# AnyLoc/AnyLoc

Hardware: NVIDIA H100
Metric: images/sec end-to-end DINOv2-VLAD descriptors (higher is better)
Workload: dtype f32-equivalent (tensor-core fp16 3-term split, fp32 accumulate)

## Files before the change

anyloc_b200/csrc/attention_wg.cu:

```cuda
#include <stdlib.h>
#include "tc_common.cuh"

namespace anyloc {
namespace awg {

using namespace tc;

__device__ __forceinline__ float ex2(float x) {
  float y; asm("ex2.approx.ftz.f32 %0, %1;" : "=f"(y) : "f"(x)); return y;
}

constexpr int BQ = 128, BKV = 64, HD = 64, THREADS = 384, STAGES = 4;
constexpr int TILE_BYTES = 64 * 128;

template <int FMT> struct Cfg {
  static constexpr int NT = Fmt<FMT>::LO ? 2 : 1;
  static constexpr int Q_BYTES = NT * 2 * TILE_BYTES;
  static constexpr int K_OFF = 0, V_OFF = NT * TILE_BYTES;
  static constexpr int STAGE_BYTES = 2 * NT * TILE_BYTES;
  static constexpr int BAR_OFF = Q_BYTES + STAGES * STAGE_BYTES;
  static constexpr int SMEM_BYTES = BAR_OFF + 256 + 1024 ;
};

template <int FMT, bool VARLEN>
__device__ __forceinline__ void attention_wg_cta(const CUtensorMap* tm_hi, const CUtensorMap* tm_lo, int T, int D,
                                                 void* __restrict__ o_hi_, void* __restrict__ o_lo_,
                                                 const VarlenAttnTable* tab) {
  using C = Cfg<FMT>;
  using F = Fmt<FMT>;
  constexpr bool PAIRS = F::LO;
  extern __shared__ uint8_t smem_raw[];
  uint8_t* smem = reinterpret_cast<uint8_t*>((reinterpret_cast<uintptr_t>(smem_raw) + 1023) & ~(uintptr_t)1023);
  uint64_t* full_bar = reinterpret_cast<uint64_t*>(smem + C::BAR_OFF);
  uint64_t* empty_bar = full_bar + STAGES;
  uint64_t* q_bar = empty_bar + STAGES;

  int qt = blockIdx.x;
  const int h = blockIdx.y;
  int img = blockIdx.z, row0 = 0;
  size_t out0 = (size_t)blockIdx.z * T;
  if constexpr (VARLEN) {
    int lo = 0, hi = tab->n - 1;
    while (lo < hi) {
      const int mid = (lo + hi + 1) >> 1;
      if (tab->tile0[mid] <= qt) lo = mid; else hi = mid - 1;
    }
    qt -= tab->tile0[lo]; T = tab->len[lo]; row0 = tab->row0[lo]; img = 0; out0 = (size_t)row0;
  }
  const int nblk = (T + BKV - 1) / BKV;
  const int active = min(2, (T - qt * BQ + 63) / 64);
  const int wg = threadIdx.x >> 7;

  if (threadIdx.x == 0) {
    asm volatile("prefetch.tensormap [%0];" ::"l"(tm_hi) : "memory");
    for (int s = 0; s < STAGES; ++s) { mbar_init(smem_u32(full_bar + s), 1); mbar_init(smem_u32(empty_bar + s), active); }
    mbar_init(smem_u32(q_bar), 1);
    asm volatile("fence.mbarrier_init.release.cluster;" ::: "memory");
  }
  __syncthreads();

  if (wg == 0) {
    setmaxnreg_dec<24>();
    if (threadIdx.x == 0) {
      const uint32_t qb = smem_u32(q_bar);
      mbar_expect_tx(qb, C::Q_BYTES);
      for (int a = 0; a < C::NT; ++a)
        for (int r = 0; r < 2; ++r)
          tma_load_3d(smem_u32(smem + (2 * a + r) * TILE_BYTES), a ? tm_lo : tm_hi, qb, h * HD,
                      row0 + qt * BQ + 64 * r, img);
      for (int j = 0; j < nblk; ++j) {
        const int stage = j % STAGES;
        mbar_wait(smem_u32(empty_bar + stage), ((j / STAGES) & 1) ^ 1);
        const uint32_t fb = smem_u32(full_bar + stage);
        mbar_expect_tx(fb, C::STAGE_BYTES);
        const uint32_t sb = smem_u32(smem + C::Q_BYTES + stage * C::STAGE_BYTES);
        for (int a = 0; a < C::NT; ++a) {
          tma_load_3d(sb + C::K_OFF + a * TILE_BYTES, a ? tm_lo : tm_hi, fb, D + h * HD, row0 + j * BKV, img);
          tma_load_3d(sb + C::V_OFF + a * TILE_BYTES, a ? tm_lo : tm_hi, fb, 2 * D + h * HD, row0 + j * BKV, img);
        }
      }
    }
    return;
  }

  setmaxnreg_inc<240>();
  const int cw = wg - 1;
  if (qt * BQ + cw * 64 >= T) return;
  const int t = threadIdx.x & 127, warp = t >> 5, lane = t & 31, g = lane >> 2, t4 = lane & 3;
  constexpr bool SCALED = F::SCALED;
  const float P_SCALE = SCALED ? 1024.0f : 1.0f;
  const float kScale = 0.125f * 1.4426950408889634f * (SCALED ? 1.0f / (kActScale * kActScale) : 1.0f);
  auto logit = [&](float s) {
    if constexpr (SCALED) return fmaf(s, kScale, s * 0.0f);
    else return s * kScale;
  };

  const uint32_t q_base = smem_u32(smem) + cw * TILE_BYTES;
  const uint64_t dq_hi = make_desc(q_base), dq_lo = make_desc(q_base + 2 * TILE_BYTES);
  auto stage_addr = [&](int j) { return smem_u32(smem + C::Q_BYTES + (j % STAGES) * C::STAGE_BYTES); };

  auto issue_s = [&](float* s, int j) {
    const uint32_t sb = stage_addr(j);
    const uint64_t dk_hi = make_desc(sb + C::K_OFF), dk_lo = make_desc(sb + C::K_OFF + TILE_BYTES);
    fence_regs<32>(s);
    wgmma_fence();
#pragma unroll
    for (int k = 0; k < 4; ++k) {
      const uint64_t adv = (uint64_t)((k * 32) >> 4);
      wgmma_m64n64_ss<FMT>(s, dq_hi + adv, dk_hi + adv, k != 0 ? 1u : 0u);
      if constexpr (PAIRS) {
        wgmma_m64n64_ss<FMT>(s, dq_lo + adv, dk_hi + adv, 1u);
        wgmma_m64n64_ss<FMT>(s, dq_hi + adv, dk_lo + adv, 1u);
      }
    }
    wgmma_commit();
    fence_regs<32>(s);
  };

  float o[32];
#pragma unroll
  for (int i = 0; i < 32; ++i) o[i] = 0.f;
  float m0 = -INFINITY, m1 = -INFINITY, l0 = 0.f, l1 = 0.f;

  auto block = [&](float* sc, float* sn, int j) {
    if (j + 1 < nblk) {
      mbar_wait(smem_u32(full_bar + (j + 1) % STAGES), ((j + 1) / STAGES) & 1);
      issue_s(sn, j + 1);
    }
    float p[32];
#pragma unroll
    for (int i = 0; i < 32; ++i) p[i] = sc[i];
    float mx0 = m0, mx1 = m1;
#pragma unroll
    for (int nt = 0; nt < 8; ++nt) {
      const int key = j * BKV + nt * 8 + 2 * t4;
#pragma unroll
      for (int e = 0; e < 2; ++e) {
        const bool live = key + e < T;
        p[4 * nt + e] = live ? logit(p[4 * nt + e]) : -INFINITY;
        p[4 * nt + 2 + e] = live ? logit(p[4 * nt + 2 + e]) : -INFINITY;
        mx0 = fmaxf(mx0, p[4 * nt + e]); mx1 = fmaxf(mx1, p[4 * nt + 2 + e]);
      }
    }
    mx0 = fmaxf(mx0, __shfl_xor_sync(0xffffffffu, mx0, 1)); mx0 = fmaxf(mx0, __shfl_xor_sync(0xffffffffu, mx0, 2));
    mx1 = fmaxf(mx1, __shfl_xor_sync(0xffffffffu, mx1, 1)); mx1 = fmaxf(mx1, __shfl_xor_sync(0xffffffffu, mx1, 2));
    const float alpha0 = ex2(m0 - mx0), alpha1 = ex2(m1 - mx1);
    m0 = mx0; m1 = mx1;
    float r0 = 0.f, r1 = 0.f;
#pragma unroll
    for (int nt = 0; nt < 8; ++nt) {
      p[4 * nt + 0] = ex2(p[4 * nt + 0] - mx0); p[4 * nt + 1] = ex2(p[4 * nt + 1] - mx0);
      p[4 * nt + 2] = ex2(p[4 * nt + 2] - mx1); p[4 * nt + 3] = ex2(p[4 * nt + 3] - mx1);
      r0 += p[4 * nt + 0] + p[4 * nt + 1]; r1 += p[4 * nt + 2] + p[4 * nt + 3];
    }
    l0 = l0 * alpha0 + r0; l1 = l1 * alpha1 + r1;

    uint32_t ph[4][4], pl[4][4];
#pragma unroll
    for (int ks = 0; ks < 4; ++ks) {
#pragma unroll
      for (int i = 0; i < 4; ++i) {
        F::pack2(p[8 * ks + 2 * i] * P_SCALE, p[8 * ks + 2 * i + 1] * P_SCALE, ph[ks][i], pl[ks][i]);
      }
    }
    const uint32_t sb = stage_addr(j);
    if constexpr (VARLEN) {
      const int rem = T - j * BKV;
      if (rem < BKV) {
        const int pieces = (BKV - rem) * 8;
        for (int i = cw * 128 + t; i < C::NT * pieces; i += active * 128) {
          const int a = i / pieces, r = rem + (i % pieces) / 8;
          asm volatile("st.shared.v4.u32 [%0], {%1, %1, %1, %1};" ::"r"(sb + C::V_OFF + a * TILE_BYTES + r * 128 +
                                                                          (i % 8) * 16), "r"(0u) : "memory");
        }
        fence_proxy_async_smem();
        named_bar_sync<1>(active * 128);
      }
    }
    const uint64_t dv_hi = make_desc_mn(sb + C::V_OFF), dv_lo = make_desc_mn(sb + C::V_OFF + TILE_BYTES);
    float pv[32];
#pragma unroll
    for (int i = 0; i < 32; ++i) pv[i] = 0.f;
    fence_regs<32>(pv);
    wgmma_fence();
#pragma unroll
    for (int ks = 0; ks < 4; ++ks) {
      const uint64_t adv = (uint64_t)((ks * 2048) >> 4);
      wgmma_m64n64_rs_tb<FMT>(pv, ph[ks], dv_hi + adv, ks != 0 ? 1u : 0u);
      if constexpr (PAIRS) {
        wgmma_m64n64_rs_tb<FMT>(pv, pl[ks], dv_hi + adv, 1u);
        wgmma_m64n64_rs_tb<FMT>(pv, ph[ks], dv_lo + adv, 1u);
      }
    }
    wgmma_commit();
    fence_regs<32>(pv);
    wgmma_wait<0>();
    fence_regs<32>(pv);
    fence_regs<32>(sn);
    if (t == 0) mbar_arrive(smem_u32(empty_bar + j % STAGES));
#pragma unroll
    for (int nd = 0; nd < 8; ++nd) {
      o[4 * nd + 0] = o[4 * nd + 0] * alpha0 + pv[4 * nd + 0]; o[4 * nd + 1] = o[4 * nd + 1] * alpha0 + pv[4 * nd + 1];
      o[4 * nd + 2] = o[4 * nd + 2] * alpha1 + pv[4 * nd + 2]; o[4 * nd + 3] = o[4 * nd + 3] * alpha1 + pv[4 * nd + 3];
    }
  };

  float sa[32], sb[32];
  mbar_wait(smem_u32(q_bar), 0);
  mbar_wait(smem_u32(full_bar), 0);
  issue_s(sa, 0);
  wgmma_wait<0>();
  fence_regs<32>(sa);
  for (int j = 0; j < nblk; j += 2) {
    block(sa, sb, j);
    if (j + 1 < nblk) block(sb, sa, j + 1);
  }

  l0 += __shfl_xor_sync(0xffffffffu, l0, 1); l0 += __shfl_xor_sync(0xffffffffu, l0, 2);
  l1 += __shfl_xor_sync(0xffffffffu, l1, 1); l1 += __shfl_xor_sync(0xffffffffu, l1, 2);
  const float inv0 = 1.0f / (l0 * P_SCALE), inv1 = 1.0f / (l1 * P_SCALE);
  const int q0 = qt * BQ + cw * 64 + warp * 16 + g;
#pragma unroll
  for (int half = 0; half < 2; ++half) {
    const int q = q0 + 8 * half;
    if (q >= T) continue;
    const float inv = half ? inv1 : inv0;
    const size_t off = (out0 + q) * (size_t)D + (size_t)h * HD + 2 * t4;
#pragma unroll
    for (int nd = 0; nd < 8; ++nd) {
      uint32_t hh, ll;
      F::pack2(o[4 * nd + 2 * half] * inv, o[4 * nd + 2 * half + 1] * inv, hh, ll);
      *reinterpret_cast<uint32_t*>(reinterpret_cast<typename F::T*>(o_hi_) + off + nd * 8) = hh;
      if constexpr (F::LO) *reinterpret_cast<uint32_t*>(reinterpret_cast<typename F::T*>(o_lo_) + off + nd * 8) = ll;
    }
  }
}

template <int FMT>
__global__ void __launch_bounds__(THREADS, 1)
attention_wg_kernel(const __grid_constant__ CUtensorMap tm_hi, const __grid_constant__ CUtensorMap tm_lo, int T, int D,
                    void* __restrict__ o_hi, void* __restrict__ o_lo) {
  attention_wg_cta<FMT, false>(&tm_hi, &tm_lo, T, D, o_hi, o_lo, nullptr);
}

template <int FMT>
__global__ void __launch_bounds__(THREADS, 1)
attention_wg_varlen_kernel(const __grid_constant__ CUtensorMap tm_hi, const __grid_constant__ CUtensorMap tm_lo,
                           const __grid_constant__ VarlenAttnTable tab, int D, void* __restrict__ o_hi,
                           void* __restrict__ o_lo) {
  attention_wg_cta<FMT, true>(&tm_hi, &tm_lo, 0, D, o_hi, o_lo, &tab);
}

static int launch(const void* qkv_hi, const void* qkv_lo, int imgs, int rows, int T, const VarlenAttnTable* tab,
                  dim3 grid, int D, void* o_hi, void* o_lo, int fmt, cudaStream_t st) {
  CUtensorMap m_hi, m_lo;
  int rc;
  if ((rc = tc::make_map_3d16(&m_hi, qkv_hi, imgs, rows, 3 * D, 64, fmt))) return rc;
  if ((rc = tc::make_map_3d16(&m_lo, format_info(fmt).lo ? qkv_lo : qkv_hi, imgs, rows, 3 * D, 64, fmt))) return rc;
  return fmt_switch(fmt, [&](auto c) {
    constexpr int FMT = decltype(c)::value;
    if constexpr (sizeof(typename Fmt<FMT>::T) != 2) {
      set_error("attention_wg: format %d is not a 2-byte format", fmt);
      return (int)ANYLOC_ERR_ARG;
    } else {
      static unsigned long long seen = 0;
      if (first_use_on_this_device(&seen)) {
        ANYLOC_CHECK_CUDA(cudaFuncSetAttribute(attention_wg_kernel<FMT>, cudaFuncAttributeMaxDynamicSharedMemorySize,
                                               Cfg<FMT>::SMEM_BYTES));
        ANYLOC_CHECK_CUDA(cudaFuncSetAttribute(attention_wg_varlen_kernel<FMT>,
                                               cudaFuncAttributeMaxDynamicSharedMemorySize, Cfg<FMT>::SMEM_BYTES));
      }
      if (tab)
        attention_wg_varlen_kernel<FMT><<<grid, THREADS, Cfg<FMT>::SMEM_BYTES, st>>>(m_hi, m_lo, *tab, D, o_hi, o_lo);
      else
        attention_wg_kernel<FMT><<<grid, THREADS, Cfg<FMT>::SMEM_BYTES, st>>>(m_hi, m_lo, T, D, o_hi, o_lo);
      ANYLOC_CHECK_LAUNCH();
      return (int)ANYLOC_OK;
    }
  });
}

}

int attention_wg_launch(const void* qkv_hi, const void* qkv_lo, int B, int T, int D, int heads, void* o_hi, void* o_lo,
                        int fmt, cudaStream_t st) {
  using namespace awg;
  return launch(qkv_hi, qkv_lo, B, T, T, nullptr, dim3(cdiv(T, BQ), heads, B), D, o_hi, o_lo, fmt, st);
}

int attention_wg_varlen_launch(const void* qkv_hi, const void* qkv_lo, const VarlenAttnTable& tab, int D, int heads,
                               void* o_hi, void* o_lo, int fmt, cudaStream_t st) {
  using namespace awg;
  VarlenAttnTable t = tab;
  int tiles = 0, rows = 0;
  for (int k = 0; k < t.n; ++k) {
    t.tile0[k] = tiles;
    tiles += cdiv(t.len[k], BQ);
    if (t.row0[k] + t.len[k] > rows) rows = t.row0[k] + t.len[k];
  }
  return launch(qkv_hi, qkv_lo, 1, rows, 0, &t, dim3(tiles, heads), D, o_hi, o_lo, fmt, st);
}

}
```

anyloc_b200/csrc/tc_common.cuh:

```cuda
#pragma once
#include <cuda.h>
#include "formats.cuh"

namespace anyloc {
namespace tc {

__device__ __forceinline__ uint32_t smem_u32(const void* p) { return (uint32_t)__cvta_generic_to_shared(p); }

__device__ __forceinline__ void mbar_init(uint32_t bar, uint32_t count) {
  asm volatile("mbarrier.init.shared::cta.b64 [%0], %1;" ::"r"(bar), "r"(count));
}
__device__ __forceinline__ void mbar_expect_tx(uint32_t bar, uint32_t bytes) {
  asm volatile("mbarrier.arrive.expect_tx.shared::cta.b64 _, [%0], %1;" ::"r"(bar), "r"(bytes) : "memory");
}
__device__ __forceinline__ void mbar_arrive(uint32_t bar) {
  asm volatile("mbarrier.arrive.shared::cta.b64 _, [%0];" ::"r"(bar) : "memory");
}
__device__ __forceinline__ void mbar_wait(uint32_t bar, uint32_t parity) {
  uint32_t done = 0;
  long long t0 = 0;
  for (uint32_t it = 0; !done; ++it) {
    asm volatile(
        "{\n\t.reg .pred p;\n\t"
        "mbarrier.try_wait.parity.shared::cta.b64 p, [%1], %2;\n\t"
        "selp.u32 %0, 1, 0, p;\n\t}"
        : "=r"(done) : "r"(bar), "r"(parity) : "memory");
    if (!done && (it & 0x3ff) == 0x3ff) {
      long long now = clock64();
      if (t0 == 0) t0 = now;
      else if (now - t0 > 8000000000LL) __trap();
    }
  }
}
__device__ __forceinline__ void tma_load_2d(uint32_t dst, const CUtensorMap* map, uint32_t bar, int c0, int c1) {
  asm volatile(
      "cp.async.bulk.tensor.2d.shared::cluster.global.mbarrier::complete_tx::bytes [%0], [%1, {%3, %4}], [%2];"
      ::"r"(dst), "l"(map), "r"(bar), "r"(c0), "r"(c1) : "memory");
}

__device__ __forceinline__ void tma_store_2d(const CUtensorMap* map, uint32_t src, int c0, int c1) {
  asm volatile("cp.async.bulk.tensor.2d.global.shared::cta.bulk_group [%0, {%2, %3}], [%1];"
               ::"l"(map), "r"(src), "r"(c0), "r"(c1) : "memory");
}
__device__ __forceinline__ void bulk_commit() { asm volatile("cp.async.bulk.commit_group;" ::: "memory"); }
template <int N>
__device__ __forceinline__ void bulk_wait_read() { asm volatile("cp.async.bulk.wait_group.read %0;" ::"n"(N) : "memory"); }
template <int N>
__device__ __forceinline__ void bulk_wait() { asm volatile("cp.async.bulk.wait_group %0;" ::"n"(N) : "memory"); }
__device__ __forceinline__ void fence_proxy_async_smem() { asm volatile("fence.proxy.async.shared::cta;" ::: "memory"); }
template <int ID>
__device__ __forceinline__ void named_bar_sync(int count) {
  asm volatile("bar.sync %0, %1;" ::"n"(ID), "r"(count) : "memory");
}

__device__ __forceinline__ uint64_t make_desc(uint32_t saddr) {
  uint64_t d = 0;
  d |= (uint64_t)((saddr & 0x3FFFF) >> 4);
  d |= (uint64_t)1 << 16;
  d |= (uint64_t)(1024 >> 4) << 32;
  d |= (uint64_t)1 << 62;
  return d;
}

__device__ __forceinline__ void wgmma_fence() { asm volatile("wgmma.fence.sync.aligned;" ::: "memory"); }
__device__ __forceinline__ void wgmma_commit() { asm volatile("wgmma.commit_group.sync.aligned;" ::: "memory"); }
template <int N>
__device__ __forceinline__ void wgmma_wait() { asm volatile("wgmma.wait_group.sync.aligned %0;" ::"n"(N) : "memory"); }
template <int R>
__device__ __forceinline__ void fence_regs(float* d) {
#pragma unroll
  for (int i = 0; i < R; ++i) asm volatile("" : "+f"(d[i])::"memory");
}

#define ANYLOC_WG_D64                                                                                               \
  "+f"(d[0]), "+f"(d[1]), "+f"(d[2]), "+f"(d[3]), "+f"(d[4]), "+f"(d[5]), "+f"(d[6]), "+f"(d[7]), "+f"(d[8]),       \
      "+f"(d[9]), "+f"(d[10]), "+f"(d[11]), "+f"(d[12]), "+f"(d[13]), "+f"(d[14]), "+f"(d[15]), "+f"(d[16]),        \
      "+f"(d[17]), "+f"(d[18]), "+f"(d[19]), "+f"(d[20]), "+f"(d[21]), "+f"(d[22]), "+f"(d[23]), "+f"(d[24]),       \
      "+f"(d[25]), "+f"(d[26]), "+f"(d[27]), "+f"(d[28]), "+f"(d[29]), "+f"(d[30]), "+f"(d[31]), "+f"(d[32]),       \
      "+f"(d[33]), "+f"(d[34]), "+f"(d[35]), "+f"(d[36]), "+f"(d[37]), "+f"(d[38]), "+f"(d[39]), "+f"(d[40]),       \
      "+f"(d[41]), "+f"(d[42]), "+f"(d[43]), "+f"(d[44]), "+f"(d[45]), "+f"(d[46]), "+f"(d[47]), "+f"(d[48]),       \
      "+f"(d[49]), "+f"(d[50]), "+f"(d[51]), "+f"(d[52]), "+f"(d[53]), "+f"(d[54]), "+f"(d[55]), "+f"(d[56]),       \
      "+f"(d[57]), "+f"(d[58]), "+f"(d[59]), "+f"(d[60]), "+f"(d[61]), "+f"(d[62]), "+f"(d[63])
#define ANYLOC_WG_D64_STR                                                                                           \
  "{%0, %1, %2, %3, %4, %5, %6, %7, %8, %9, %10, %11, %12, %13, %14, %15, %16, %17, %18, %19, %20, %21, %22, %23, " \
  "%24, %25, %26, %27, %28, %29, %30, %31, %32, %33, %34, %35, %36, %37, %38, %39, %40, %41, %42, %43, %44, %45, "  \
  "%46, %47, %48, %49, %50, %51, %52, %53, %54, %55, %56, %57, %58, %59, %60, %61, %62, %63}"
#define ANYLOC_WG_M64N128(SHAPE_TYPES, TAIL)                                                                        \
  asm volatile("{\n\t.reg .pred p;\n\tsetp.ne.b32 p, %66, 0;\n\t"                                                 \
               "wgmma.mma_async.sync.aligned.m64n128" SHAPE_TYPES " " ANYLOC_WG_D64_STR ", %64, %65, p, 1, 1" TAIL     \
               ";\n\t}"                                                                                              \
               : ANYLOC_WG_D64 : "l"(adesc), "l"(bdesc), "r"(scale_d))

template <int FMT>
__device__ __forceinline__ void wgmma_m64n128(float* d, uint64_t adesc, uint64_t bdesc, uint32_t scale_d) {
  if constexpr (FMT == ANYLOC_PAIR_TF32) ANYLOC_WG_M64N128("k8.f32.tf32.tf32", "");
  else if constexpr (FMT == ANYLOC_PAIR_FP8) ANYLOC_WG_M64N128("k32.f32.e4m3.e4m3", "");
  else if constexpr (FMT == ANYLOC_PAIR_BF16) ANYLOC_WG_M64N128("k16.f32.bf16.bf16", ", 0, 0");
  else ANYLOC_WG_M64N128("k16.f32.f16.f16", ", 0, 0");
}
#undef ANYLOC_WG_M64N128
#undef ANYLOC_WG_D64
#undef ANYLOC_WG_D64_STR

__device__ __forceinline__ void tma_load_3d(uint32_t dst, const CUtensorMap* map, uint32_t bar, int c0, int c1, int c2) {
  asm volatile(
      "cp.async.bulk.tensor.3d.shared::cluster.global.mbarrier::complete_tx::bytes [%0], [%1, {%3, %4, %5}], [%2];"
      ::"r"(dst), "l"(map), "r"(bar), "r"(c0), "r"(c1), "r"(c2) : "memory");
}

template <int N> __device__ __forceinline__ void setmaxnreg_dec() { asm volatile("setmaxnreg.dec.sync.aligned.u32 %0;" ::"n"(N)); }
template <int N> __device__ __forceinline__ void setmaxnreg_inc() { asm volatile("setmaxnreg.inc.sync.aligned.u32 %0;" ::"n"(N)); }

__device__ __forceinline__ uint64_t make_desc_mn(uint32_t saddr) {
  uint64_t d = 0;
  d |= (uint64_t)((saddr & 0x3FFFF) >> 4);
  d |= (uint64_t)(1024 >> 4) << 16;
  d |= (uint64_t)(1024 >> 4) << 32;
  d |= (uint64_t)1 << 62;
  return d;
}

#define ANYLOC_WG_D32                                                                                               \
  "+f"(d[0]), "+f"(d[1]), "+f"(d[2]), "+f"(d[3]), "+f"(d[4]), "+f"(d[5]), "+f"(d[6]), "+f"(d[7]), "+f"(d[8]),       \
      "+f"(d[9]), "+f"(d[10]), "+f"(d[11]), "+f"(d[12]), "+f"(d[13]), "+f"(d[14]), "+f"(d[15]), "+f"(d[16]),        \
      "+f"(d[17]), "+f"(d[18]), "+f"(d[19]), "+f"(d[20]), "+f"(d[21]), "+f"(d[22]), "+f"(d[23]), "+f"(d[24]),       \
      "+f"(d[25]), "+f"(d[26]), "+f"(d[27]), "+f"(d[28]), "+f"(d[29]), "+f"(d[30]), "+f"(d[31])
#define ANYLOC_WG_D32_STR                                                                                           \
  "{%0, %1, %2, %3, %4, %5, %6, %7, %8, %9, %10, %11, %12, %13, %14, %15, %16, %17, %18, %19, %20, %21, %22, %23, " \
  "%24, %25, %26, %27, %28, %29, %30, %31}"

template <int FMT>
__device__ __forceinline__ void wgmma_m64n64_ss(float* d, uint64_t adesc, uint64_t bdesc, uint32_t scale_d) {
  if constexpr (FMT == ANYLOC_PAIR_BF16)
    asm volatile("{\n\t.reg .pred p;\n\tsetp.ne.b32 p, %34, 0;\n\t"
                 "wgmma.mma_async.sync.aligned.m64n64k16.f32.bf16.bf16 " ANYLOC_WG_D32_STR ", %32, %33, p, 1, 1, 0, 0;\n\t}"
                 : ANYLOC_WG_D32 : "l"(adesc), "l"(bdesc), "r"(scale_d));
  else
    asm volatile("{\n\t.reg .pred p;\n\tsetp.ne.b32 p, %34, 0;\n\t"
                 "wgmma.mma_async.sync.aligned.m64n64k16.f32.f16.f16 " ANYLOC_WG_D32_STR ", %32, %33, p, 1, 1, 0, 0;\n\t}"
                 : ANYLOC_WG_D32 : "l"(adesc), "l"(bdesc), "r"(scale_d));
}

template <int FMT>
__device__ __forceinline__ void wgmma_m64n64_rs_tb(float* d, const uint32_t* a, uint64_t bdesc, uint32_t scale_d) {
  if constexpr (FMT == ANYLOC_PAIR_BF16)
    asm volatile("{\n\t.reg .pred p;\n\tsetp.ne.b32 p, %37, 0;\n\t"
                 "wgmma.mma_async.sync.aligned.m64n64k16.f32.bf16.bf16 " ANYLOC_WG_D32_STR
                 ", {%32, %33, %34, %35}, %36, p, 1, 1, 1;\n\t}"
                 : ANYLOC_WG_D32 : "r"(a[0]), "r"(a[1]), "r"(a[2]), "r"(a[3]), "l"(bdesc), "r"(scale_d));
  else
    asm volatile("{\n\t.reg .pred p;\n\tsetp.ne.b32 p, %37, 0;\n\t"
                 "wgmma.mma_async.sync.aligned.m64n64k16.f32.f16.f16 " ANYLOC_WG_D32_STR
                 ", {%32, %33, %34, %35}, %36, p, 1, 1, 1;\n\t}"
                 : ANYLOC_WG_D32 : "r"(a[0]), "r"(a[1]), "r"(a[2]), "r"(a[3]), "l"(bdesc), "r"(scale_d));
}
#undef ANYLOC_WG_D32
#undef ANYLOC_WG_D32_STR

int make_map(CUtensorMap* map, const void* ptr, int rows, int K, int ld, int box_rows, int fmt);
int make_map_3d16(CUtensorMap* map, const void* ptr, int imgs, int rows, int cols, int box_rows, int fmt);

}
}
```

Before: 179.0.

## Hold Q in registers and defer PV wait to overlap with next softmax

Loads the Q tile once into registers with ldmatrix and switches the QK^T wgmma from shared-memory A operands to register A operands. It also restructures the flash-attention loop so the PV wgmma of block j is not waited on immediately. The output accumulation for block j is deferred into block j+1, after the next S result is ready, so PV matmul overlaps with the next softmax. This adds register pressure from 32 extra Q registers and a persistent pv buffer, and makes the stage-release timing more delicate.

```diff
diff --git a/anyloc_b200/csrc/attention_wg.cu b/anyloc_b200/csrc/attention_wg.cu
--- a/anyloc_b200/csrc/attention_wg.cu
+++ b/anyloc_b200/csrc/attention_wg.cu
@@ -95,9 +95,20 @@
     else return s * kScale;
   };
 
-  const uint32_t q_base = smem_u32(smem) + cw * TILE_BYTES;
-  const uint64_t dq_hi = make_desc(q_base), dq_lo = make_desc(q_base + 2 * TILE_BYTES);
   auto stage_addr = [&](int j) { return smem_u32(smem + C::Q_BYTES + (j % STAGES) * C::STAGE_BYTES); };
+
+  uint32_t qh[4][4], ql[4][4];
+  mbar_wait(smem_u32(q_bar), 0);
+  {
+    const int r = warp * 16 + (lane & 7) + ((lane >> 3) & 1) * 8;
+    const uint32_t q_row = smem_u32(smem) + cw * TILE_BYTES + r * 128;
+#pragma unroll
+    for (int ks = 0; ks < 4; ++ks) {
+      const uint32_t off = (uint32_t)(((2 * ks + (lane >> 4)) ^ (r & 7)) << 4);
+      ldsm_x4(qh[ks], q_row + off);
+      if constexpr (PAIRS) ldsm_x4(ql[ks], q_row + 2 * TILE_BYTES + off);
+    }
+  }
 
   auto issue_s = [&](float* s, int j) {
     const uint32_t sb = stage_addr(j);
@@ -107,10 +118,10 @@
 #pragma unroll
     for (int k = 0; k < 4; ++k) {
       const uint64_t adv = (uint64_t)((k * 32) >> 4);
-      wgmma_m64n64_ss<FMT>(s, dq_hi + adv, dk_hi + adv, k != 0 ? 1u : 0u);
+      wgmma_m64n64_rs<FMT, 0>(s, qh[k], dk_hi + adv, k != 0 ? 1u : 0u);
       if constexpr (PAIRS) {
-        wgmma_m64n64_ss<FMT>(s, dq_lo + adv, dk_hi + adv, 1u);
-        wgmma_m64n64_ss<FMT>(s, dq_hi + adv, dk_lo + adv, 1u);
+        wgmma_m64n64_rs<FMT, 0>(s, ql[k], dk_hi + adv, 1u);
+        wgmma_m64n64_rs<FMT, 0>(s, qh[k], dk_lo + adv, 1u);
       }
     }
     wgmma_commit();
@@ -118,15 +129,32 @@
   };
 
   float o[32];
+  float pv[32];
 #pragma unroll
   for (int i = 0; i < 32; ++i) o[i] = 0.f;
   float m0 = -INFINITY, m1 = -INFINITY, l0 = 0.f, l1 = 0.f;
+  float alpha0 = 1.f, alpha1 = 1.f;
+
+  auto update_o = [&](int j) {
+    fence_regs<32>(pv);
+    if (t == 0) mbar_arrive(smem_u32(empty_bar + j % STAGES));
+#pragma unroll
+    for (int nd = 0; nd < 8; ++nd) {
+      o[4 * nd + 0] = o[4 * nd + 0] * alpha0 + pv[4 * nd + 0]; o[4 * nd + 1] = o[4 * nd + 1] * alpha0 + pv[4 * nd + 1];
+      o[4 * nd + 2] = o[4 * nd + 2] * alpha1 + pv[4 * nd + 2]; o[4 * nd + 3] = o[4 * nd + 3] * alpha1 + pv[4 * nd + 3];
+    }
+  };
 
   auto block = [&](float* sc, float* sn, int j) {
     if (j + 1 < nblk) {
       mbar_wait(smem_u32(full_bar + (j + 1) % STAGES), ((j + 1) / STAGES) & 1);
       issue_s(sn, j + 1);
-    }
+      wgmma_wait<1>();
+    } else {
+      wgmma_wait<0>();
+    }
+    fence_regs<32>(sc);
+    if (j > 0) update_o(j - 1);
     float p[32];
 #pragma unroll
     for (int i = 0; i < 32; ++i) p[i] = sc[i];
@@ -144,7 +172,7 @@
     }
     mx0 = fmaxf(mx0, __shfl_xor_sync(0xffffffffu, mx0, 1)); mx0 = fmaxf(mx0, __shfl_xor_sync(0xffffffffu, mx0, 2));
     mx1 = fmaxf(mx1, __shfl_xor_sync(0xffffffffu, mx1, 1)); mx1 = fmaxf(mx1, __shfl_xor_sync(0xffffffffu, mx1, 2));
-    const float alpha0 = ex2(m0 - mx0), alpha1 = ex2(m1 - mx1);
+    alpha0 = ex2(m0 - mx0); alpha1 = ex2(m1 - mx1);
     m0 = mx0; m1 = mx1;
     float r0 = 0.f, r1 = 0.f;
 #pragma unroll
@@ -178,7 +206,6 @@
       }
     }
     const uint64_t dv_hi = make_desc_mn(sb + C::V_OFF), dv_lo = make_desc_mn(sb + C::V_OFF + TILE_BYTES);
-    float pv[32];
 #pragma unroll
     for (int i = 0; i < 32; ++i) pv[i] = 0.f;
     fence_regs<32>(pv);
@@ -186,35 +213,25 @@
 #pragma unroll
     for (int ks = 0; ks < 4; ++ks) {
       const uint64_t adv = (uint64_t)((ks * 2048) >> 4);
-      wgmma_m64n64_rs_tb<FMT>(pv, ph[ks], dv_hi + adv, ks != 0 ? 1u : 0u);
+      wgmma_m64n64_rs<FMT, 1>(pv, ph[ks], dv_hi + adv, ks != 0 ? 1u : 0u);
       if constexpr (PAIRS) {
-        wgmma_m64n64_rs_tb<FMT>(pv, pl[ks], dv_hi + adv, 1u);
-        wgmma_m64n64_rs_tb<FMT>(pv, ph[ks], dv_lo + adv, 1u);
+        wgmma_m64n64_rs<FMT, 1>(pv, pl[ks], dv_hi + adv, 1u);
+        wgmma_m64n64_rs<FMT, 1>(pv, ph[ks], dv_lo + adv, 1u);
       }
     }
     wgmma_commit();
     fence_regs<32>(pv);
-    wgmma_wait<0>();
-    fence_regs<32>(pv);
-    fence_regs<32>(sn);
-    if (t == 0) mbar_arrive(smem_u32(empty_bar + j % STAGES));
-#pragma unroll
-    for (int nd = 0; nd < 8; ++nd) {
-      o[4 * nd + 0] = o[4 * nd + 0] * alpha0 + pv[4 * nd + 0]; o[4 * nd + 1] = o[4 * nd + 1] * alpha0 + pv[4 * nd + 1];
-      o[4 * nd + 2] = o[4 * nd + 2] * alpha1 + pv[4 * nd + 2]; o[4 * nd + 3] = o[4 * nd + 3] * alpha1 + pv[4 * nd + 3];
-    }
   };
 
   float sa[32], sb[32];
-  mbar_wait(smem_u32(q_bar), 0);
   mbar_wait(smem_u32(full_bar), 0);
   issue_s(sa, 0);
-  wgmma_wait<0>();
-  fence_regs<32>(sa);
   for (int j = 0; j < nblk; j += 2) {
     block(sa, sb, j);
     if (j + 1 < nblk) block(sb, sa, j + 1);
   }
+  wgmma_wait<0>();
+  update_o(nblk - 1);
 
   l0 += __shfl_xor_sync(0xffffffffu, l0, 1); l0 += __shfl_xor_sync(0xffffffffu, l0, 2);
   l1 += __shfl_xor_sync(0xffffffffu, l1, 1); l1 += __shfl_xor_sync(0xffffffffu, l1, 2);
diff --git a/anyloc_b200/csrc/tc_common.cuh b/anyloc_b200/csrc/tc_common.cuh
--- a/anyloc_b200/csrc/tc_common.cuh
+++ b/anyloc_b200/csrc/tc_common.cuh
@@ -129,30 +129,23 @@
   "{%0, %1, %2, %3, %4, %5, %6, %7, %8, %9, %10, %11, %12, %13, %14, %15, %16, %17, %18, %19, %20, %21, %22, %23, " \
   "%24, %25, %26, %27, %28, %29, %30, %31}"
 
-template <int FMT>
-__device__ __forceinline__ void wgmma_m64n64_ss(float* d, uint64_t adesc, uint64_t bdesc, uint32_t scale_d) {
-  if constexpr (FMT == ANYLOC_PAIR_BF16)
-    asm volatile("{\n\t.reg .pred p;\n\tsetp.ne.b32 p, %34, 0;\n\t"
-                 "wgmma.mma_async.sync.aligned.m64n64k16.f32.bf16.bf16 " ANYLOC_WG_D32_STR ", %32, %33, p, 1, 1, 0, 0;\n\t}"
-                 : ANYLOC_WG_D32 : "l"(adesc), "l"(bdesc), "r"(scale_d));
-  else
-    asm volatile("{\n\t.reg .pred p;\n\tsetp.ne.b32 p, %34, 0;\n\t"
-                 "wgmma.mma_async.sync.aligned.m64n64k16.f32.f16.f16 " ANYLOC_WG_D32_STR ", %32, %33, p, 1, 1, 0, 0;\n\t}"
-                 : ANYLOC_WG_D32 : "l"(adesc), "l"(bdesc), "r"(scale_d));
-}
-
-template <int FMT>
-__device__ __forceinline__ void wgmma_m64n64_rs_tb(float* d, const uint32_t* a, uint64_t bdesc, uint32_t scale_d) {
+template <int FMT, int TRANS_B>
+__device__ __forceinline__ void wgmma_m64n64_rs(float* d, const uint32_t* a, uint64_t bdesc, uint32_t scale_d) {
   if constexpr (FMT == ANYLOC_PAIR_BF16)
     asm volatile("{\n\t.reg .pred p;\n\tsetp.ne.b32 p, %37, 0;\n\t"
                  "wgmma.mma_async.sync.aligned.m64n64k16.f32.bf16.bf16 " ANYLOC_WG_D32_STR
-                 ", {%32, %33, %34, %35}, %36, p, 1, 1, 1;\n\t}"
-                 : ANYLOC_WG_D32 : "r"(a[0]), "r"(a[1]), "r"(a[2]), "r"(a[3]), "l"(bdesc), "r"(scale_d));
+                 ", {%32, %33, %34, %35}, %36, p, 1, 1, %38;\n\t}"
+                 : ANYLOC_WG_D32 : "r"(a[0]), "r"(a[1]), "r"(a[2]), "r"(a[3]), "l"(bdesc), "r"(scale_d), "n"(TRANS_B));
   else
     asm volatile("{\n\t.reg .pred p;\n\tsetp.ne.b32 p, %37, 0;\n\t"
                  "wgmma.mma_async.sync.aligned.m64n64k16.f32.f16.f16 " ANYLOC_WG_D32_STR
-                 ", {%32, %33, %34, %35}, %36, p, 1, 1, 1;\n\t}"
-                 : ANYLOC_WG_D32 : "r"(a[0]), "r"(a[1]), "r"(a[2]), "r"(a[3]), "l"(bdesc), "r"(scale_d));
+                 ", {%32, %33, %34, %35}, %36, p, 1, 1, %38;\n\t}"
+                 : ANYLOC_WG_D32 : "r"(a[0]), "r"(a[1]), "r"(a[2]), "r"(a[3]), "l"(bdesc), "r"(scale_d), "n"(TRANS_B));
+}
+
+__device__ __forceinline__ void ldsm_x4(uint32_t* r, uint32_t saddr) {
+  asm volatile("ldmatrix.sync.aligned.m8n8.x4.shared.b16 {%0, %1, %2, %3}, [%4];"
+               : "=r"(r[0]), "=r"(r[1]), "=r"(r[2]), "=r"(r[3]) : "r"(saddr) : "memory");
 }
 #undef ANYLOC_WG_D32
 #undef ANYLOC_WG_D32_STR
```

After: 179.4, median of 6. About the same (+0.2%).
